# pauxy-qmc/pauxy

Hardware: AMD Instinct MI355X
Metric: walker_steps_per_sec (higher is better)
Workload: dtype f64; 1 GPU; generic Cholesky AFQMC: Nbasis=100, Nchol=500, RHF trial 25+25 electrons, 256 walkers/GPU, dt=0.005, reortho/10, comb/5, energy/10 (BASELINE configs[2]); walkers_total=256, rng=device-philox, population_control=device comb (one rank)

## Files before the change

include/afqmc_hip.h:

```cpp
#ifndef AFQMC_HIP_H
#define AFQMC_HIP_H

#include <stdint.h>

#ifdef __cplusplus
extern "C" {
#endif

typedef struct afq_handle afq_handle;

#define AFQ_OK            0
#define AFQ_EINVAL       (-1)
#define AFQ_ESTATE       (-2)
#define AFQ_EHIP         (-3)
#define AFQ_ENOMEM       (-4)
#define AFQ_EUNSUPPORTED (-5)
#define AFQ_EWEIGHT      (-6)
#define AFQ_EOVERFLOW    (-7)
#define AFQ_ECOMM        (-8)

#define AFQ_SYS_GENERIC 1
#define AFQ_SYS_HUBBARD 2
#define AFQ_SYS_UEG     3

// ... 48 lines not shown
                       const double *vqvec, double vol, const double *H1diag, double ecore);
int afq_set_trial(afq_handle *h, const double *psi);
int afq_set_propagator_hirsch(afq_handle *h, const double *bt2, double dt, int charge_decomposition);
int afq_hirsch_free_projection(afq_handle *h, int on);
int afq_hirsch_single_site(afq_handle *h, int on);
int afq_propagate_hirsch_free(afq_handle *h, const double *u, int32_t *fields_out, double eshift);
int afq_propagate_hirsch(afq_handle *h, double eshift);
int afq_hirsch_kinetic(afq_handle *h);
int afq_hirsch_two_body(afq_handle *h, const double *u, int32_t *fields_out, int32_t *used_out);
int afq_hirsch_finish(afq_handle *h, double eshift);

int afq_local_energy_full_g(afq_handle *h, const double *G, int n, double *E_out);
int afq_ueg_pair_sums(afq_handle *h, const double *G, int n, double *E_out, double *two_rdm_out);
int afq_hubbard_energy_full_g(afq_handle *h, const double *G, int n, double *E_out);

int afq_bp_configure(afq_handle *h, int nbp);
int afq_bp_steps(afq_handle *h, int32_t *steps_out);
int afq_bp_update(afq_handle *h, const double *phi_bp0, int nstblz, int restore_weights, int eval_energy,
                  int reset, double *est_out);
int afq_bp_observables(afq_handle *h, int two_rdm, int ekt, const double *h1, const double *L, int nL);
int afq_bp_ekt_chunks(afq_handle *h, int nc, int ncy);
int afq_bp_update_ext(afq_handle *h, const double *phi_bp0, int nstblz, int restore_weights, int eval_energy,
                      int reset, double *est_out, double *two_rdm_out, double *fock_out);
int afq_bp_update_msd(afq_handle *h, int ndet, const double *dets, const double *coeffs, int nstblz, int restore_weights,
                      int eval_energy, int reset, double *est_out, double *detw_out);

int afq_itcf_configure(afq_handle *h, int nmax, int neqlb, int stable, int restore_weights);
int afq_itcf_update(afq_handle *h, const double *psi_T, int nstblz, double *spgf_out, double *denom_out);

int afq_set_trial_multi(afq_handle *h, int ndet, const double *psi, const double *coeffs, const double *rchol);
int afq_walkers_det_weights(afq_handle *h, double *weights_out);

int afq_set_propagator(afq_handle *h, const double *BH1, const double *mf_shift,
                       double dt, int exp_order, int flags);

int afq_walkers_alloc(afq_handle *h, int nw);
int afq_walkers_set(afq_handle *h, int field, const void *host, int first, int count);
int afq_walkers_get(afq_handle *h, int field, void *host, int first, int count);
int afq_walkers_device_ptr(afq_handle *h, int field, void **dev_ptr, int64_t *bytes_per_walker);

int afq_greens(afq_handle *h, int want_G, double *ovlp_out);
int afq_calc_overlap(afq_handle *h, double *ovlp_out);
int afq_inverse_overlap(afq_handle *h, double *oinv_out, double *ovlp_out);
int afq_propagate(afq_handle *h, const double *xi, double eshift_re, double eshift_im);
int afq_propagate_begin(afq_handle *h, const double *xi);
int afq_propagate_finish(afq_handle *h, double eshift_re, double eshift_im);
int afq_reortho(afq_handle *h, double *detR_out);
int afq_set_log_shift(afq_handle *h, int on, double log_shift, double detR_shift);
int afq_log_ovlp_sums(afq_handle *h, double *sums3);
int afq_local_energy(afq_handle *h, double *E_out);

int afq_set_exchange_algorithm(afq_handle *h, int mode);
int afq_exchange_algorithm(afq_handle *h, int *mode_out);

int afq_set_msd_force_bias(afq_handle *h, int mode);
int afq_msd_force_bias(afq_handle *h, int *mode_out);

int afq_force_bias(afq_handle *h, double *xbar_out);
int afq_shift_fields(afq_handle *h, const double *xi, const double *xbar,
                     double *xs_out, double *cmf_out, double *cfb_out);
int afq_vhs(afq_handle *h, const double *xs, double *vhs_out);
int afq_vhs_count(afq_handle *h, int *nv);
int afq_apply_exponential(afq_handle *h, const double *vhs);
int afq_kinetic(afq_handle *h);

int afq_cap_weights(afq_handle *h, double frac, double total_weight);
int afq_set_weight_cap(afq_handle *h, double frac, double total_weight);
int afq_popcontrol_comb(afq_handle *h, double r, double target_weight,
                        int32_t *parent_ix, double *total_weight_out);

#define AFQ_COMM_ID_BYTES 128
#define AFQ_COMM_NSTATS 12
typedef int (*afq_allgather_fn)(const void *send, void *recv, int bytes, void *user);
int afq_comm_unique_id(void *id_out);
int afq_comm_available(void);
int afq_comm_init(afq_handle *h, const void *unique_id, int rank, int nranks);
int afq_comm_init_ipc(afq_handle *h, int rank, int nranks, afq_allgather_fn allgather, void *user);
int afq_comm_destroy(afq_handle *h);
int afq_comm_set_transport(afq_handle *h, int window);
int afq_comm_set_capacity(afq_handle *h, int max_walkers_per_peer);
int afq_comm_set_timeout(afq_handle *h, double seconds);
int afq_comm_probe(afq_handle *h, int64_t *mismatch_out);
int afq_comm_stats(afq_handle *h, int64_t *out);
int afq_comm_parent_ix(afq_handle *h, int32_t *parent_ix_global);
int afq_estimates_allreduce(afq_handle *h, double *buf, int nest);
int afq_comm_init_local(afq_handle **handles, int n);
int afq_popcontrol_comb_local(afq_handle **handles, int n, double r, double target_weight,
                              int32_t *parent_ix_global, double *total_weight_out);
int afq_estimates_allreduce_local(afq_handle **handles, int n);
int afq_walkers_scale_weights(afq_handle *h, double scale);
int afq_walkers_copy(afq_handle *h, int src, int dst);
int afq_walker_pack_bytes(afq_handle *h, int64_t *bytes);
int afq_walker_pack(afq_handle *h, int iw, void *dev_buf);
int afq_walker_unpack(afq_handle *h, int iw, const void *dev_buf);
int afq_walkers_reset_weights(afq_handle *h);
int afq_estimates_update(afq_handle *h, int eval_energy);
int afq_estimates_rdm(afq_handle *h, int on);
int afq_estimates_sf(afq_handle *h, int on);
int afq_estimates_sf_get(afq_handle *h, double *sf_out , int zero);
int afq_estimates_rdm_get(afq_handle *h, double *rdm_out , int zero);
int afq_estimates_get(afq_handle *h, double *est_out , int zero);
int afq_estimates_fuse_next(afq_handle *h);
int afq_estimates_get_begin(afq_handle *h, int zero);
int afq_estimates_update_publish(afq_handle *h, int eval_energy, int zero);
int afq_estimates_get_end(afq_handle *h, double *est_out );

// ... 30 lines not shown
```

pauxy_amd/_lib.py:

```python
import ctypes
import os
from ctypes import POINTER, c_char_p, c_double, c_int, c_int32, c_int64, c_uint64, c_void_p

HERE = os.path.dirname(os.path.abspath(__file__))
LIB_PATH = os.environ.get("AFQ_LIBRARY") or os.path.join(HERE, "libafqmc_hip.so")

AFQ_OK = 0
AFQ_EWEIGHT, AFQ_EOVERFLOW, AFQ_ECOMM = -6, -7, -8
AFQ_COMM_NSTATS = 12
ALLGATHER_FN = ctypes.CFUNCTYPE(ctypes.c_int, ctypes.c_void_p, ctypes.c_void_p, ctypes.c_int, ctypes.c_void_p)
AFQ_SYS_GENERIC, AFQ_SYS_HUBBARD, AFQ_SYS_UEG = 1, 2, 3
AFQ_PROP_HYBRID, AFQ_PROP_FORCE_BIAS, AFQ_PROP_FREE_PROJECTION, AFQ_PROP_HUBBARD_SPIN = 1, 2, 4, 8
(F_PHI, F_WEIGHT, F_UNSCALED_WEIGHT, F_OT, F_HYBRID_ENERGY, F_PHASE, F_DETR, F_ELOC, F_GHALF, F_G,
 F_XBAR, F_XSHIFTED, F_ENERGY, F_LOG_DETR) = range(14)

_h = c_void_p
_dp = c_void_p
_ip = c_void_p

SIGNATURES = {
    "afq_version": [],
    "afq_create": [c_int, POINTER(_h)],
    "afq_destroy": [_h],
    "afq_last_error": [_h],
# ... 46 lines not shown
    "afq_rng_seed": [_h, c_uint64, c_uint64],
    "afq_counters": [_h, c_void_p, c_int],
    "afq_counters_ext": [_h, c_void_p, c_int, c_int],
    "afq_propagator_issued_flops": [_h, POINTER(c_double), POINTER(c_double)],
    "afq_timers": [_h, _dp, c_int],
    "afq_enable_timers": [_h, c_int],
    "afq_stream": [_h, POINTER(c_void_p)],
    "afq_inverse_overlap": [_h, _dp, _dp],
    "afq_set_propagator_hirsch": [_h, _dp, c_double, c_int],
    "afq_propagate_hirsch": [_h, c_double],
    "afq_hirsch_free_projection": [_h, c_int],
    "afq_hirsch_single_site": [_h, c_int],
    "afq_propagate_hirsch_free": [_h, _dp, c_void_p, c_double],
    "afq_hirsch_kinetic": [_h],
    "afq_hirsch_two_body": [_h, _dp, _dp, _dp],
    "afq_hirsch_finish": [_h, c_double],
    "afq_bp_configure": [_h, c_int],
    "afq_bp_steps": [_h, _dp],
    "afq_bp_update": [_h, _dp, c_int, c_int, c_int, c_int, _dp],
    "afq_bp_observables": [_h, c_int, c_int, _dp, _dp, c_int],
    "afq_bp_ekt_chunks": [_h, c_int, c_int],
    "afq_bp_update_ext": [_h, _dp, c_int, c_int, c_int, c_int, _dp, _dp, _dp],
    "afq_bp_update_msd": [_h, c_int, _dp, _dp, c_int, c_int, c_int, c_int, _dp, _dp],
    "afq_itcf_configure": [_h, c_int, c_int, c_int, c_int],
    "afq_itcf_update": [_h, _dp, c_int, _dp, _dp],
    "afq_local_energy_full_g": [_h, _dp, c_int, _dp],
    "afq_ueg_pair_sums": [_h, _dp, c_int, _dp, _dp],
    "afq_hubbard_energy_full_g": [_h, _dp, c_int, _dp],
    "afq_set_trial_multi": [_h, c_int, _dp, _dp, _dp],
    "afq_walkers_det_weights": [_h, _dp],
    "afq_rng_normal": [_h, _dp, c_int64],
    "afq_rng_philox4x32": [_h, c_void_p, c_void_p, c_int],
    "afq_debug": [_h, c_int, c_int],
    "afq_last_launch": [_h, c_void_p, c_int, POINTER(c_uint64), POINTER(c_uint64)],
    "afq_comm_unique_id": [c_void_p],
    "afq_comm_available": [],
    "afq_comm_init": [_h, c_void_p, c_int, c_int],
    "afq_comm_init_ipc": [_h, c_int, c_int, ALLGATHER_FN, c_void_p],
    "afq_comm_set_transport": [_h, c_int],
    "afq_comm_probe": [_h, c_void_p],
    "afq_comm_destroy": [_h],
    "afq_comm_set_capacity": [_h, c_int],
    "afq_comm_set_timeout": [_h, c_double],
    "afq_launch_trace": [_h, c_int],
    "afq_launch_trace_get": [_h, c_void_p, c_int, c_void_p, c_void_p, c_int, POINTER(c_int)],
    "afq_comm_stats": [_h, c_void_p],
    "afq_comm_parent_ix": [_h, c_void_p],
    "afq_estimates_allreduce": [_h, _dp, c_int],
    "afq_comm_init_local": [POINTER(_h), c_int],
    "afq_popcontrol_comb_local": [POINTER(_h), c_int, c_double, c_double, c_void_p, POINTER(c_double)],
    "afq_estimates_allreduce_local": [POINTER(_h), c_int],
    "afq_set_exchange_algorithm": [_h, c_int],
    "afq_exchange_algorithm": [_h, POINTER(c_int)],
    "afq_set_msd_force_bias": [_h, c_int],
    "afq_msd_force_bias": [_h, POINTER(c_int)],
    "afq_kernel_trace": [_h, c_int],
    "afq_kernel_trace_stride": [_h, c_int, c_int],
    "afq_kernel_trace_get": [_h, c_int, _dp, c_int, POINTER(c_int)],
    "afq_kernel_issued_flops": [_h, c_int, POINTER(c_double)],
}


class AfqLibraryError(RuntimeError):
    pass


class AfqError(RuntimeError):
    def __init__(self, code, text):
        RuntimeError.__init__(self, "libafqmc_hip error %d: %s" % (code, text))
        self.code = code


_lib = None


def load(path=None):
    global _lib
    if _lib is not None and path is None:
        return _lib
    p = path or LIB_PATH
    if not os.path.exists(p):
        raise AfqLibraryError(
            "%s not found: build it with `python -c 'import __graft_entry__ as g; g.build()'` "
            "(or `make -C pauxy_amd/csrc`).  There is no CPU fallback." % p)
    try:
        lib = ctypes.CDLL(p)
    except OSError as e:
        raise AfqLibraryError("cannot load %s: %s" % (p, e))
    for name, args in SIGNATURES.items():
        try:
            fn = getattr(lib, name)
        except AttributeError:
            raise AfqLibraryError("%s does not export %s" % (p, name))
        fn.argtypes = args
        fn.restype = c_char_p if name == "afq_last_error" else c_int
    if path is None:
        _lib = lib
    return lib

K_PROPAGATOR, K_EXCHANGE, K_VHS, K_FORCE_BIAS, K_GREENS = range(5)
```

pauxy_amd/csrc/afq_api.hip:

```cpp
#include <algorithm>
#include <cmath>
#include <complex>
#include <cstdio>
#include <cstdlib>
#include <cstring>
#include "afq_host.h"

namespace {

void free_dets(afq_handle *h) {
    h->mem.release(LT_TRIAL);
    h->dets.assign(1, afq_handle::DetOps());
    h->ndet = 1;
    select_det(h, 0, true);
    h->msd_fb_gbar = false;
}

void free_system(afq_handle *h) {
    free_dets(h);
    h->mem.release(LT_SYSTEM);
    h->hs_cplx = 0; h->sf_nlong = 0; h->kind = 0;
    h->hirsch = false;
}

// ... 921 lines not shown
    const bool keep = kept != GreensCache::NOTHING && h->ndet == 1;
    bool scaled = false;
    { PhaseTimer t(h, T_QR); if ((rc = k_reortho(h, keep ? h->ovlp_new : nullptr, &scaled))) return rc; }
    if (keep) {
        if (!scaled && (rc = k_scale_by_inverse(h, h->ovlp_new, h->detR))) return rc;
        h->gf.keep(kept);
    }
    if (h->log_shift_on && (rc = k_log_shift_reortho(h))) return rc;
    return copy_out(h, detR_out, h->detR, sizeof(double) * h->nw);
}

static int local_energy_dets(afq_handle *h) {
    cplx *final_e = h->energy;
    int rc = AFQ_OK;
    for (int d = 0; d < h->ndet && !rc; ++d) {
        select_det(h, d);
        h->energy = h->energy_all + (size_t)d * 3 * h->nw;
        rc = k_energy_generic(h);
    }
    h->energy = final_e;
    select_det(h, 0);
    return rc;
}

static int local_energy(afq_handle *h) {
    if (h->kind == AFQ_SYS_GENERIC && h->ndet > 1) {
        int rc = local_energy_dets(h);
        if (rc) return rc;
        return k_msd_energy_combine(h);
    }
    if (h->kind == AFQ_SYS_GENERIC) return k_energy_generic(h);
    if (h->kind == AFQ_SYS_HUBBARD) return k_energy_hubbard(h);
    if (!h->G) AFQ_FAIL(h, AFQ_ESTATE, "afq_greens must run before afq_local_energy");
    return k_energy_ueg(h);
}

int afq_local_energy(afq_handle *h, double *E_out) {
    AFQ_API(h, "afq_local_energy");
    if (!h) return AFQ_EINVAL;
    int rc = need_ready(h, false);
    if (rc) return rc;
    if (!h->rH1 && h->kind != AFQ_SYS_UEG) AFQ_FAIL(h, AFQ_ESTATE, "half-rotated H1 missing (set trial)");
    if ((rc = ensure_spin_ghalf(h))) return rc;
    { PhaseTimer t(h, T_ENERGY); if ((rc = local_energy(h))) return rc; }
    return copy_out(h, E_out, h->energy, sizeof(cplx) * 3 * h->nw);
}

int afq_set_exchange_algorithm(afq_handle *h, int mode) {
    if (!h || mode < 0 || mode > 2) return AFQ_EINVAL;
    h->exx_mode = mode;
    return AFQ_OK;
}

int afq_set_msd_force_bias(afq_handle *h, int mode) {
    if (!h || mode < 0 || mode > 2) return AFQ_EINVAL;
    h->msd_fb_mode = mode;
    return AFQ_OK;
}

int afq_msd_force_bias(afq_handle *h, int *mode) {
    if (!h || !mode) return AFQ_EINVAL;
    if (h->kind != AFQ_SYS_GENERIC || !h->have_trial || !h->nw) AFQ_FAIL(h, AFQ_ESTATE, "generic system, trial and walkers must be set");
    *mode = h->ndet <= 1 ? 0 : k_msd_gbar_wanted(h) ? 2 : 1;
    return AFQ_OK;
}

int afq_exchange_algorithm(afq_handle *h, int *mode) {
    if (!h || !mode) return AFQ_EINVAL;
    if (h->kind != AFQ_SYS_GENERIC || !h->have_trial) AFQ_FAIL(h, AFQ_ESTATE, "generic system and trial must be set");
    *mode = k_exchange_uses_quadratic(h) ? 2 : 1;
    return AFQ_OK;
}

int afq_force_bias(afq_handle *h, double *xbar_out) {
    if (!h) return AFQ_EINVAL;
    int rc = need_ready(h, true);
    if (rc) return rc;
    if ((rc = force_bias(h))) return rc;
    return copy_out(h, xbar_out, h->xbar, sizeof(cplx) * (size_t)h->nw * h->K);
}

int afq_shift_fields(afq_handle *h, const double *xi, const double *xbar, double *xs_out, double *cmf_out,
                     double *cfb_out) {
    if (!h || !xi || !xbar) return AFQ_EINVAL;
    int rc = need_ready(h, true);
    if (rc) return rc;
    const size_t n = (size_t)h->nw * h->K;
    AFQ_HIP(h, hipMemcpyAsync(h->xi, xi, sizeof(double) * n, hipMemcpyHostToDevice, h->stream));
    AFQ_HIP(h, hipMemcpyAsync(h->xbar, xbar, sizeof(cplx) * n, hipMemcpyHostToDevice, h->stream));
    if ((rc = k_fields_explicit(h, h->xi, h->xbar, h->xs, h->cmf, h->cfb))) return rc;
    if ((rc = copy_out(h, xs_out, h->xs, sizeof(cplx) * n))) return rc;
    if ((rc = copy_out(h, cmf_out, h->cmf, sizeof(cplx) * h->nw))) return rc;
    return copy_out(h, cfb_out, h->cfb, sizeof(cplx) * h->nw);
}

int afq_vhs_count(afq_handle *h, int *nv) {
    if (!h || !nv) return AFQ_EINVAL;
    *nv = h->nv;
    return AFQ_OK;
}

int afq_vhs(afq_handle *h, const double *xs, double *vhs_out) {
    if (!h || !xs || !vhs_out) return AFQ_EINVAL;
    int rc = need_ready(h, true);
    if (rc) return rc;
    const size_t n = (size_t)h->nw * h->K;
// ... 685 lines not shown
```

pauxy_amd/csrc/afq_internal.h:

```cpp
#pragma once
#include <hip/hip_runtime.h>
#include <stdint.h>
#include <cstdlib>
#include <string>
#include <vector>
#include "../../include/afqmc_hip.h"
#include "greens_cache.h"
#include "dev_mem.h"

typedef double2 cplx;

__host__ __device__ inline cplx cmake(double r, double i) { return make_double2(r, i); }
__host__ __device__ inline cplx cadd(cplx a, cplx b) { return cmake(a.x + b.x, a.y + b.y); }
__host__ __device__ inline cplx csub(cplx a, cplx b) { return cmake(a.x - b.x, a.y - b.y); }
__host__ __device__ inline cplx cmul(cplx a, cplx b) {
    return cmake(a.x * b.x - a.y * b.y, a.x * b.y + a.y * b.x);
}
__host__ __device__ inline cplx cconj(cplx a) { return cmake(a.x, -a.y); }
__host__ __device__ inline cplx cscale(cplx a, double s) { return cmake(a.x * s, a.y * s); }
__host__ __device__ inline void cfma(cplx &a, cplx b, cplx c) {
    a.x = fma(b.x, c.x, a.x); a.x = fma(-b.y, c.y, a.x);
    a.y = fma(b.x, c.y, a.y); a.y = fma(b.y, c.x, a.y);
}
__host__ __device__ inline double cabs2(cplx a) { return a.x * a.x + a.y * a.y; }
__device__ inline cplx cdiv(cplx a, cplx b) {
    if (fabs(b.x) >= fabs(b.y)) {
        double r = b.y / b.x, d = b.x + b.y * r;
        return cmake((a.x + a.y * r) / d, (a.y - a.x * r) / d);
    } else {
        double r = b.x / b.y, d = b.x * r + b.y;
        return cmake((a.x * r + a.y) / d, (a.y * r - a.x) / d);
    }
}

#define AFQ_NSCAL 12
enum { AFQ_HS_HERMITIAN = 1, AFQ_HS_GENERAL = 2 };
enum { T_GREENS = 0, T_ONEBODY, T_FB, T_VHS, T_EXP, T_OVLP, T_QR, T_ENERGY, T_COUNT };

#define AFQ_NCOUNTERS 8

struct afq_handle {
    int device = 0;
    hipStream_t stream = nullptr;
    std::string err;
    DevMem mem;

    int kind = 0;
    int M = 0, K = 0, na = 0, nb = 0, nt = 0;
    double ecore = 0.0;
    double *hs_pot = nullptr;
    bool hs_sym = false;
    double *L_full = nullptr;
    int2 *hs_pair = nullptr;
    int hs_cplx = 0;
    double *hs_pot_im = nullptr;
    int2 *hs_pair_im = nullptr;
    long ld_hs_im = 0;
    cplx *L_full_c = nullptr;
    long ld_hs = 0, ld_rc = 0;
    bool rchol_real = true;
    double *rchol_re = nullptr;
    double *rchol_im = nullptr;
    double *rchol_frag[2] = {nullptr, nullptr};
    double *rchol_frag_im[2] = {nullptr, nullptr};
    void *atil[2] = {nullptr, nullptr};
    bool atil_unavailable = false;
    bool rchol_same = false;
    int exx_mode = 0;
    cplx *exq_y = nullptr;
    size_t exq_y_len = 0;
    cplx *H1 = nullptr;
    cplx *rH1 = nullptr;
    double U = 0.0;
    int nq = 0;
    int64_t nnzA = 0, nnzB = 0;
    int64_t *iA_colptr = nullptr, *iA_row = nullptr; cplx *iA_val = nullptr;
    int64_t *iB_colptr = nullptr, *iB_row = nullptr; cplx *iB_val = nullptr;
    int64_t *iA_rowptr = nullptr, *iA_col = nullptr; cplx *iA_rval = nullptr;
    int64_t *iB_rowptr = nullptr, *iB_col = nullptr; cplx *iB_rval = nullptr;
    int ell_len = 0; int *ell_row = nullptr; cplx *ell_val = nullptr;
    int ueg_nrows = 0; int *ueg_rmap = nullptr; int *ueg_rows = nullptr;
    int *ueg_kp = nullptr, *ueg_pm = nullptr, *ueg_koff = nullptr, *ueg_poff = nullptr;
    int64_t *kpq_off = nullptr, *kpq_i = nullptr, *kpq_kpq = nullptr;
    int64_t *pmq_off = nullptr, *pmq_i = nullptr, *pmq_pmq = nullptr;
    double *vqvec = nullptr; double vol = 1.0; double *H1diag = nullptr;
    void *ueg_fast = nullptr;
    int *sf_kp = nullptr, *sf_pm = nullptr, *sf_order = nullptr;
    int sf_nlong = 0;
    cplx *sf_ws = nullptr, *sf_two = nullptr;
    size_t sf_ws_len = 0, sf_two_len = 0;

    bool have_trial = false;
    cplx *psi = nullptr;
    cplx *psic = nullptr;
    cplx *psicT = nullptr;
    long psi_stride = 0;
    bool psi_real = false;
    bool psi_closed = false;
    unsigned long long *closed_bad = nullptr;
    unsigned long long closed_epoch = 0;
    unsigned long long closed_epoch_pub = 0;
    bool exx_open_hint = false;
    int *closed_w = nullptr;
    size_t closed_w_n = 0;
    bool closed_large = false;

    struct DetOps {
        cplx *psi = nullptr, *psic = nullptr, *rH1 = nullptr;
        double *rchol_re = nullptr, *rchol_im = nullptr;
        double *rchol_frag[2] = {nullptr, nullptr}, *rchol_frag_im[2] = {nullptr, nullptr};
        void *atil[2] = {nullptr, nullptr};
        bool rchol_same = false;
        GreensCache::Stamp vbias_stamp;
    };
    int ndet = 1, cur_det = 0;
    std::vector<DetOps> dets = std::vector<DetOps>(1);
    cplx *coeffs = nullptr;
    cplx *detd = nullptr;
    cplx *detd_a = nullptr;
    cplx *detw = nullptr;
    cplx *ghalf_all = nullptr;
// ... 245 lines not shown
    }
}

struct PhaseTimer {
    afq_handle *h; int slot;
    PhaseTimer(afq_handle *h_, int s) : h(h_), slot(s) {
        if (h->timers_on) hipEventRecord(h->ev0, h->stream);
    }
    ~PhaseTimer() {
        if (h->timers_on) {
            hipEventRecord(h->ev1, h->stream);
            hipEventSynchronize(h->ev1);
            float ms = 0; hipEventElapsedTime(&ms, h->ev0, h->ev1);
            h->t_ms[slot] += ms;
        }
    }
};

template <class T> struct Lent {
    T &slot; T saved;
    Lent(T &s, T v) : slot(s), saved(s) { slot = v; }
    ~Lent() { slot = saved; }
    Lent(const Lent &) = delete;
    Lent &operator=(const Lent &) = delete;
};

struct KernelTrace {
    afq_handle *h; int kind, idx;
    KernelTrace(afq_handle *h_, int k) : h(h_), kind(k), idx(-1) {
        if (!(h->ktrace_mask >> k & 1) || h->ktrace_used[k] >= 4096) return;
        if (h->ktrace_seen[k]++ % h->ktrace_stride[k]) return;
        idx = h->ktrace_used[k];
        std::vector<hipEvent_t> &ev = h->ktrace_ev[k];
        while ((int)ev.size() < 2 * idx + 2) { hipEvent_t e; hipEventCreate(&e); ev.push_back(e); }
        hipEventRecord(ev[2 * idx], h->stream);
    }
    ~KernelTrace() {
        if (idx < 0) return;
        hipEventRecord(h->ktrace_ev[kind][2 * idx + 1], h->stream);
        h->ktrace_used[kind] = idx + 1;
    }
};

int k_onebody(afq_handle *h, const cplx *rowscale = nullptr);
int k_force_bias_generic(afq_handle *h);
bool k_msd_vbias_current(afq_handle *h);
bool k_msd_gbar_wanted(afq_handle *h);
int k_force_bias_msd_gbar(afq_handle *h);
bool k_fb_use_sum(afq_handle *h);
int k_vhs_generic(afq_handle *h);
int k_apply_exponential(afq_handle *h, const cplx *vhs);
int k_full_G(afq_handle *h);
int k_prop_fused_supported(afq_handle *h);
int k_prop_fused(afq_handle *h);
int k_hirsch_alive(afq_handle *h, int mode);
int k_hirsch_kinetic(afq_handle *h);
int k_hirsch_two_body(afq_handle *h);
int k_hirsch_eshift(afq_handle *h, double fac);
int k_hirsch_free(afq_handle *h, double eshift);
int k_rng_uniform(afq_handle *h, double *u, long n);
int k_energy_full_g(afq_handle *h, const cplx *G_dev, int ng, cplx *E_dev);
int k_fullg_expand(afq_handle *h);
int k_bp_observables(afq_handle *h, int restore, cplx *two_out, cplx *fock_out);
int k_itcf_fields(afq_handle *h, cplx *xs, int t);
int k_itcf_generic_b(afq_handle *h, const cplx *vhs, const cplx *BT2, const cplx *BT2inv, cplx *B, cplx *Binv, cplx *ws,
                     cplx *detm, int *dete);
int k_itcf_hirsch_b(afq_handle *h, int t, const cplx *BT2, const cplx *BT2inv, cplx *B, cplx *Binv, double *f);
int k_itcf_mul(afq_handle *h, const cplx *A, const cplx *B, cplx *C);
int k_itcf_propagate(afq_handle *h, const cplx *B, const cplx *src, cplx *dst);
int k_itcf_projectors(afq_handle *h, const cplx *G, cplx *P, cplx *Q);
int k_itcf_weights(afq_handle *h, int restore, cplx *wfac, cplx *denom);
int k_itcf_accumulate(afq_handle *h, const cplx *Ggr, const cplx *Gls, const cplx *wfac, cplx *spgf_tau);
int k_greens_big_supported(afq_handle *h);
int k_greens_big(afq_handle *h, cplx *ghalf, cplx *det, cplx *oinv, const GreensRequest &req, GreensResult *res);
int k_reortho_big(afq_handle *h);
int k_gj_inverse(afq_handle *h, cplx *O, int n, int batch, cplx *detm, int *dete);
int k_alive(afq_handle *h);
int k_greens(afq_handle *h, cplx *det_out, const GreensRequest &req = GreensRequest(), GreensResult *res = nullptr);
int k_overlap(afq_handle *h, cplx *det_out, const GreensRequest &req = GreensRequest(), GreensResult *res = nullptr);
int k_inverse_overlap(afq_handle *h, cplx *oinv, cplx *det_out);
int k_fields(afq_handle *h);
int k_fields_explicit(afq_handle *h, const double *xi_d, const cplx *xbar_d, cplx *xs_d, cplx *cmf_d, cplx *cfb_d);
int k_xbar(afq_handle *h);
int k_bp_push(afq_handle *h);
int k_bp_fields(afq_handle *h, int i);
int k_bp_init(afq_handle *h, const cplx *phi0_dev);
int k_conj_copy(afq_handle *h, const cplx *src, cplx *dst, long n);
int k_conj_transpose(afq_handle *h, const cplx *A, cplx *At);
int k_bp_accumulate(afq_handle *h, int restore, int with_energy);
int k_bp_reset(afq_handle *h, bool first);
int k_bp_hirsch_step(afq_handle *h, int i);
int k_bp_msd_onebody(afq_handle *h, int ndet, const cplx *src, cplx *dst);
int k_bp_msd_taylor(afq_handle *h, int ndet, const cplx *vhs, cplx *phi, cplx *t0, cplx *t1);
int k_bp_msd_logr(afq_handle *h, const double *detR, double *logr, long n);
int k_bp_msd_detw(afq_handle *h, int ndet, int d, const cplx *coeffs, const double *logr, const cplx *ovlp, cplx *detw,
                  cplx *S);
int k_bp_msd_gsum(afq_handle *h, int ndet, int d, const cplx *detw, const cplx *G, cplx *gsum, const cplx *E, cplx *esum);
int k_bp_msd_finish(afq_handle *h, int ndet, int restore, cplx *detw, const cplx *S, cplx *fac);
int k_bp_msd_accumulate(afq_handle *h, const cplx *gsum, const cplx *fac, const cplx *esum, cplx *est);
int k_xbar_fields(afq_handle *h, cplx *hubbard_factors = nullptr);
int k_msd_combine(afq_handle *h, cplx *det_out, bool skip_small);
int k_msd_energy_combine(afq_handle *h);
int k_update_weight(afq_handle *h, cplx eshift);
struct WeightArgs;
WeightArgs k_weight_args(afq_handle *h, cplx eshift);
int k_reortho(afq_handle *h, cplx *keep = nullptr, bool *keep_done = nullptr);
// ... 52 lines not shown
```

pauxy_amd/csrc/k_fused.hip:

```cpp
#include <cstdlib>
#include <type_traits>

#include "mfma_gemm_wg.h"

#define PF_D 3
#ifndef PF_NW
#define PF_NW 8
#endif
#define PF_NT (64 * PF_NW)
#ifndef PF_LW
#define PF_LW PF_NW
#endif
#define PF_FPW (16 / PF_LW)

struct PropFusedArgs {
    int M, na, nb, nt, order;
    int vhs_upper;
    int same_b;
    int b_real;
    int rem4;
    int hyb;
    int symcols;
    int closed_try;
    int contig;
    const cplx *BH1;
    const cplx *vhs;
    cplx *phi;
    const int *alive;
    const void *zero16;
    unsigned long long *n_closed;
};

__device__ inline d2_t lds_read_c(unsigned addr) { return lds_read_b128(addr); }

template <int OFF> __device__ inline d2_t lds_read_off(unsigned addr) {
    d2_t v;
    asm volatile("ds_read_b128 %0, %1 offset:%2" : "=v"(v) : "v"(addr), "n"(OFF));
    return v;
}
__device__ __attribute__((always_inline)) inline d2_t lds_read_frag(unsigned base, int idx) {
    switch (idx) {
    case 0: return lds_read_off<0>(base);
    case 1: return lds_read_off<1024>(base);
    case 2: return lds_read_off<2048>(base);
    case 3: return lds_read_off<3072>(base);
    case 4: return lds_read_off<4096>(base);
    case 5: return lds_read_off<5120>(base);
    case 6: return lds_read_off<6144>(base);
    default: return lds_read_off<7168>(base);
    }
}

template <int OFF> __device__ inline double lds_read_re_off(unsigned addr) {
    double v;
    asm volatile("ds_read_b64 %0, %1 offset:%2" : "=v"(v) : "v"(addr), "n"(OFF));
    return v;
}
__device__ __attribute__((always_inline)) inline double lds_read_frag_re(unsigned base, int idx) {
    switch (idx) {
    case 0: return lds_read_re_off<0>(base);
    case 1: return lds_read_re_off<1024>(base);
    case 2: return lds_read_re_off<2048>(base);
    case 3: return lds_read_re_off<3072>(base);
    case 4: return lds_read_re_off<4096>(base);
    case 5: return lds_read_re_off<5120>(base);
    case 6: return lds_read_re_off<6144>(base);
    default: return lds_read_re_off<7168>(base);
    }
}

__device__ inline void lds_barrier() {
    asm volatile("s_waitcnt lgkmcnt(0)" ::: "memory");
    __builtin_amdgcn_s_barrier();
    asm volatile("" ::: "memory");
}

template <bool NARROW, int FULL>
__global__ __launch_bounds__(PF_NT) void prop_fused_kernel(PropFusedArgs a) {
    extern __shared__ __align__(16) unsigned char smem[];
    const int w = blockIdx.x;
    if (!a.alive[w]) return;
    const int tid = threadIdx.x, lane = tid & 63, wave = __builtin_amdgcn_readfirstlane(tid >> 6);
    const int lr = lane & 15, lk = lane >> 4;
    const int M = a.M, nt = a.nt;
    const int NCH = (M + 7) >> 3;
    const int nrt = (M + 15) >> 4;
    unsigned char *Tf = smem;
    unsigned char *ring = smem + (size_t)NCH * 8192;
    const unsigned tf_l = lds_addr(Tf), ring_l = lds_addr(ring);
    cplx *phi = a.phi + (long)w * M * nt;
    const cplx *vhs = a.vhs + (long)w * M * M;

    const int nob = a.same_b ? 1 : 2;
    const int nphase = 2 * nob + a.order;
    const int G = nphase * NCH;
    const long MM = (long)M * M;
    int gi = 0, gi_phase = 0, gi_c = 0, gi_slot = 0;
    const void *nsrc[PF_FPW];
    bool prepared = false;
    const bool refills = wave >= PF_NW - PF_LW;
    const int lw = wave - (PF_NW - PF_LW);
    const int p_row0 = (lw >> 1) * 16 + lr;
    const int p_kl = 2 * lk + (lw & 1);
    auto prepare = [&]() __attribute__((always_inline)) {
        if (!refills) { prepared = true; return; }
        const bool in_v = gi_phase >= nob && gi_phase < nob + a.order;
        const int spin = gi_phase < nob ? gi_phase : gi_phase - nob - a.order;
        const cplx *A = in_v ? vhs : a.BH1 + (spin == 1 ? MM : 0L);
        const bool sym_phase = a.vhs_upper && in_v;
        const bool live = gi < G;
        const int k = gi_c * 8 + p_kl;
#pragma unroll
        for (int t = 0; t < PF_FPW; ++t) {
            const int row = p_row0 + t * (PF_LW / 2) * 16;
            const int off = (sym_phase && k < row) ? k * M + row : row * M + k;
            nsrc[t] = (live && row < M && k < M) ? (const void *)(A + off) : a.zero16;
            asm volatile("" : "+v"(nsrc[t]));
        }
        ++gi;
        const bool wrap = gi_c + 1 == NCH;
        gi_c = wrap ? 0 : gi_c + 1;
        gi_phase += wrap ? 1 : 0;
        prepared = true;
    };
    auto issueA = [&]() __attribute__((always_inline)) {
        if (!refills) return;
        if (!prepared) prepare();
        unsigned char *dst = ring + (size_t)gi_slot * 16384;
#pragma unroll
        for (int t = 0; t < PF_FPW; ++t) glds16(nsrc[t], dst + (lw + t * PF_LW) * 1024);
        if (++gi_slot == PF_D) gi_slot = 0;
        prepared = false;
    };
    issueA(); issueA();
    prepare();
    bool closed = false;
    if (a.closed_try) {
        bool same = true;
        for (int p = tid >> 5; p < M; p += PF_NT / 32) {
            const int c = tid & 31;
            if (c < a.na) {
                const cplx x = phi[p * nt + c], y = phi[p * nt + a.na + c];
                same = same && __double_as_longlong(x.x) == __double_as_longlong(y.x) &&
                       __double_as_longlong(x.y) == __double_as_longlong(y.y);
            }
        }
        closed = __builtin_amdgcn_readfirstlane(__syncthreads_and(same ? 1 : 0)) != 0;
        if (closed && tid == 0) atomicAdd(a.n_closed, 1ULL);
    }
    const bool relayout = closed && a.contig;
    const int contig = relayout ? 0 : a.contig, hyb = relayout ? 0 : a.hyb;
    const int sym_n = (a.symcols && !relayout) ? a.na : 0;
    auto wcol = [&](const int c) -> int {
        if (!sym_n) return c;
        if (c < 16) return c;
        if (c < 32) return sym_n + (c - 16);
        if (c < 40) return 16 + (c - 32);
        if (c < 48) return sym_n + 16 + (c - 40);
        const int e = c - 48, extra = sym_n - 24;
        return e < extra ? 24 + e : sym_n + 24 + (e - extra);
    };

    for (int e = tid; e < NCH * 512; e += PF_NT) {
        const int j = e & 15, kk = (e >> 4) & 3, pb = (e >> 6) & 1, slot = (e >> 7) & 3, ch = e >> 9;
        const int p = ch * 8 + 2 * kk + pb, sp = contig ? 0 : slot >> 1, col = (contig ? slot : slot & 1) * 16 + j;
        const int ns_ = contig ? nt : sp ? a.nb : a.na, off_ = sp ? a.na : 0;
        const bool ok = p < M && col < ns_;
        const cplx v = phi[ok ? p * nt + off_ + wcol(col) : 0];
        ((d2_t *)Tf)[e] = ok ? (d2_t){v.x, v.y} : (d2_t){0.0, 0.0};
    }
    __syncthreads();

    auto t_ok = [&](int ti, int r) -> bool { return 2 * ti + (r >> 1) < NCH; };
    const unsigned t_lane = (unsigned)((lk & 1) * 1024 + ((lk >> 1) * 16 + lr) * 16);
    auto t_addr = [&](int ti, int r, int cs) -> unsigned {
        unsigned base = t_lane;
        asm volatile("" : "+v"(base));
        return base + (unsigned)(((2 * ti * 4 + cs) * 2) * 1024) + (unsigned)((r >> 1) * 8192 + (r & 1) * 512);
    };

    int ring_slot = 0;
    auto next_chunk = [&]() __attribute__((always_inline)) -> unsigned {
        asm volatile("s_waitcnt vmcnt(%0)" ::"n"((PF_D - 2) * PF_FPW) : "memory");
        __builtin_amdgcn_s_barrier();
        issueA();
        const unsigned sl = ring_l + ring_slot * 16384;
        if (++ring_slot == PF_D) ring_slot = 0;
        return sl;
    };
    auto next_chunk_sync = [&]() __attribute__((always_inline)) -> unsigned {
        asm volatile("s_waitcnt vmcnt(%0)" ::"n"((PF_D - 2) * PF_FPW) : "memory");
        __builtin_amdgcn_s_barrier();
        const unsigned sl = ring_l + ring_slot * 16384;
        ring_slot = ring_slot + 1 == PF_D ? 0 : ring_slot + 1;
        return sl;
    };

    auto one_body = [&](auto nsl_tag, int slot0, bool to_global, auto real_tag, const int rt) __attribute__((always_inline)) {
        constexpr int NSL = decltype(nsl_tag)::value;
        constexpr bool BR = decltype(real_tag)::value;
        constexpr int SS = (NARROW && FULL) ? 2 : 1;
// ... 710 lines not shown
        else if (nrt <= 6) taylor(I2{}, I1{}, std::true_type{}, 4 + (wave & 1), 2 * ((wave - 4) >> 1), 1, std::false_type{});
        else taylor(I2{}, I1{}, std::true_type{}, (wave & 1) ? 6 : 4, 2 * ((wave - 4) >> 1), (wave & 1) ? 1 : 2, std::false_type{});
    }
    else if (FULL == 7 && contig) {
        if constexpr (FULL == 7) {
            using I1 = std::integral_constant<int, 1>;
            using I2 = std::integral_constant<int, 2>;
            auto deal = [&](auto nu) __attribute__((always_inline)) {
                if (wave == 0 || wave == 2) taylor(I2{}, I2{}, std::false_type{}, wave, 0, 2, std::false_type{});
                else if (wave == 1 || wave == 3) taylor_h(std::true_type{}, std::false_type{}, nu, wave - 1, 2, 3, 0);
                else if (wave == 4 || wave == 6) taylor(I1{}, I1{}, std::true_type{}, 4, (wave - 4) >> 1, 1, std::true_type{});
                else if (wave == 5) taylor(I1{}, I2{}, std::true_type{}, 5, 0, 1, std::false_type{});
                else taylor_h(std::true_type{}, std::true_type{}, nu, 4, 2, 3, 2);
            };
            if (hyb == 2) deal(I2{});
            else deal(I1{});
        }
    }
    else if (FULL >= 5 && closed) {
        using I1 = std::integral_constant<int, 1>;
        using I2 = std::integral_constant<int, 2>;
        const int cs = wave & 1;
        if (wave < 4) taylor(I2{}, I1{}, std::false_type{}, 2 * (wave >> 1), cs, 2, std::false_type{});
        else if constexpr (FULL == 7) {
            if (a.rem4) {
                if (wave < 6) taylor(I1{}, I1{}, std::true_type{}, 4, cs, 1, std::true_type{});
                else taylor(I1{}, I1{}, std::true_type{}, 5, cs, 1, std::false_type{});
            } else {
                if (wave < 6) taylor(I2{}, I1{}, std::true_type{}, 4, cs, 2, std::false_type{});
                else taylor(I1{}, I1{}, std::true_type{}, 6, cs, 1, std::false_type{});
            }
        }
        else taylor(I1{}, I1{}, std::true_type{}, (FULL == 6 && wave >= 6) ? 5 : 4, cs, 1, std::false_type{});
        mirror_spin();
    }
    else if (wave < 4) taylor(std::integral_constant<int, 2>{}, std::integral_constant<int, 2>{}, std::false_type{}, 2 * (wave >> 1), 2 * (wave & 1), 2, std::false_type{});
    else if constexpr (FULL == 7) {
        if (a.rem4) taylor(std::integral_constant<int, 2>{}, std::integral_constant<int, 1>{}, std::true_type{}, 4, wave - 4, 2, std::true_type{});
        else taylor(std::integral_constant<int, 3>{}, std::integral_constant<int, 1>{}, std::true_type{}, 4, wave - 4, 3, std::false_type{});
    }
    else if (FULL >= 5) taylor(std::integral_constant<int, FULL >= 5 ? FULL - 4 : 1>{}, std::integral_constant<int, 1>{}, std::true_type{}, 4, wave - 4, FULL - 4, std::false_type{});
    else taylor(std::integral_constant<int, 3>{}, std::integral_constant<int, 1>{}, std::true_type{}, 4, wave - 4, 3, std::false_type{});
#endif
    if (a.order == 0) lds_barrier();

    one_body_stage(true);
    asm volatile("s_waitcnt vmcnt(0)" ::: "memory");
}

int k_prop_fused_supported(afq_handle *h) {
    return !h->vhs_diag && h->nv == 1 && h->M <= 104 && h->na <= 32 && h->nb <= 32 && h->nb > 0;
}

int k_prop_fused(afq_handle *h) {
    PropFusedArgs a;
    a.M = h->M; a.na = h->na; a.nb = h->nb; a.nt = h->nt; a.order = h->exp_order;
    a.vhs_upper = h->vhs_upper ? 1 : 0;
    a.same_b = h->bh1_same ? 1 : 0;
    a.b_real = h->bh1_real ? 1 : 0;
    a.rem4 = (h->M > 96 && h->M <= 100) ? 1 : 0;
    a.hyb = 0;
    a.contig = 0; a.symcols = 0;
    if (a.rem4 && a.same_b && h->na > 16 && h->nb > 16 && h->nt > 48 && h->nt <= 56 && PF_NW == 8) {
        a.contig = 1;
        a.hyb = (h->nt - 48 + 3) / 4;
    }
    a.symcols = (a.contig && h->na == h->nb) ? 1 : 0;
    a.closed_try = 0;
    a.BH1 = h->BH1; a.vhs = h->vhs; a.phi = h->phi; a.alive = h->alive; a.zero16 = h->zero_page;
    a.n_closed = h->counters + 3;
    const int NCH = (h->M + 7) / 8;
    const size_t lds = (size_t)NCH * 8192 + (size_t)PF_D * 16384;
    static size_t lds_set[6][AFQ_MAX_DEVICES] = {{0}, {0}, {0}, {0}, {0}, {0}};
    const bool narrow = h->na <= 16 && h->nb <= 16;
    KernelTrace kt(h, AFQ_K_PROPAGATOR);
    {
        const int nrt_ = (h->M + 15) / 16, ct = (h->na + 15) / 16 + (h->nb + 15) / 16;
        const double ksteps = 2.0 * NCH;
        const double per_pass = ksteps * (2048.0 * (a.rem4 ? nrt_ - 1 : nrt_) * ct + 512.0 * (a.rem4 ? ct : 0));
        const double taylor_pass = a.contig ? ksteps * (2048.0 * (nrt_ - 1) * 3 + 512.0 * (nrt_ - 1) * a.hyb + 512.0 * 4) : per_pass;
        h->issued_flops[AFQ_K_PROPAGATOR] = (3.0 * h->exp_order * taylor_pass + 2.0 * (a.b_real ? 2.0 : 3.0) * per_pass) * h->nw;
        h->prop_issued_open = h->issued_flops[AFQ_K_PROPAGATOR] / h->nw;
        const int cta = (h->na + 15) / 16;
        const double closed_pass = ksteps * (2048.0 * (a.rem4 ? nrt_ - 1 : nrt_) * cta + 512.0 * (a.rem4 ? cta : 0));
        h->prop_issued_closed = 3.0 * h->exp_order * closed_pass + 2.0 * (a.b_real ? 2.0 : 3.0) * per_pass;
    }
    const int nrt = (h->M + 15) / 16;
    const bool nofull = PF_NW != 8;
    const int full = nofull ? 0 : narrow ? (nrt == 6 ? 6 : 0) : (nrt >= 5 && h->na > 16 && h->nb > 16 ? nrt : 0);
    a.closed_try = (a.same_b && h->na == h->nb && h->exp_order > 0 && full != 0 && PF_NW == 8 &&
                    (!a.contig || a.symcols)) ? 1 : 0;
#define PF_LAUNCH_(NARROW_, FULL_, SLOT_)                                                                     \
    do {                                                                                                      \
        AFQ_HIP(h, afq_raise_lds((const void *)prop_fused_kernel<NARROW_, FULL_>, lds, lds_set[SLOT_]));      \
        AFQ_LAUNCH(h, (prop_fused_kernel<NARROW_, FULL_>), dim3(h->nw), dim3(PF_NT), lds, h->stream, a);      \
    } while (0)
    if (narrow && full) PF_LAUNCH_(true, 6, 0);
    else if (narrow) PF_LAUNCH_(true, 0, 1);
    else if (full == 7) PF_LAUNCH_(false, 7, 2);
    else if (full == 6) PF_LAUNCH_(false, 6, 3);
    else if (full == 5) PF_LAUNCH_(false, 5, 4);
    else PF_LAUNCH_(false, 0, 5);
#undef PF_LAUNCH_
    AFQ_POST(h);
    return AFQ_OK;
}
```

pauxy_amd/device.py:

```python
import ctypes

import numpy

from pauxy_amd import _lib as L


def _c128(a, shape=None):
    a = numpy.ascontiguousarray(a, dtype=numpy.complex128)
    if shape is not None:
        assert a.shape == tuple(shape), (a.shape, shape)
    return a


def _f64(a, shape=None):
    a = numpy.ascontiguousarray(a, dtype=numpy.float64)
    if shape is not None:
        assert a.shape == tuple(shape), (a.shape, shape)
    return a


def _i64(a):
    return numpy.ascontiguousarray(a, dtype=numpy.int64)


# ... 528 lines not shown
                         'reortho', 'energy'], out))

    def kernel_trace(self, on=True, kinds=None):
        arg = int(bool(on))
        if on and kinds is not None:
            arg = sum(2 << int(k) for k in kinds)
        self._ck(self.lib.afq_kernel_trace(self.h, arg))

    def kernel_trace_stride(self, kind, stride):
        self._ck(self.lib.afq_kernel_trace_stride(self.h, int(kind), int(stride)))

    def kernel_trace_get(self, kind, max_n=4096):
        out = numpy.zeros(max_n, dtype=numpy.float64)
        n = ctypes.c_int()
        self._ck(self.lib.afq_kernel_trace_get(self.h, int(kind), _p(out), max_n, ctypes.byref(n)))
        return out[:min(n.value, max_n)]

    def launch_trace(self, on=True):
        self._ck(self.lib.afq_launch_trace(self.h, int(bool(on))))

    def launch_trace_get(self):
        cap = 256
        names = ctypes.create_string_buffer(cap * 96)
        ms = numpy.zeros(cap, dtype=numpy.float64)
        cnt = numpy.zeros(cap, dtype=numpy.int64)
        n = ctypes.c_int()
        self._ck(self.lib.afq_launch_trace_get(self.h, ctypes.cast(names, ctypes.c_void_p), len(names), _p(ms), _p(cnt),
                                               cap, ctypes.byref(n)))
        out, at = {}, 0
        for k in range(min(n.value, cap)):
            end = names.raw.index(b'\0', at)
            out[names.raw[at:end].decode()] = (int(cnt[k]), float(ms[k]))
            at = end + 1
        return out

    def kernel_issued_flops(self, kind):
        out = ctypes.c_double(0.0)
        self._ck(self.lib.afq_kernel_issued_flops(self.h, int(kind), ctypes.byref(out)))
        return float(out.value)

    def propagator_issued_flops(self):
        a, b = ctypes.c_double(0.0), ctypes.c_double(0.0)
        self._ck(self.lib.afq_propagator_issued_flops(self.h, ctypes.byref(a), ctypes.byref(b)))
        return float(a.value), float(b.value)

    def set_exchange_algorithm(self, mode):
        self._ck(self.lib.afq_set_exchange_algorithm(self.h, int(mode)))

    def exchange_algorithm(self):
        m = ctypes.c_int()
        self._ck(self.lib.afq_exchange_algorithm(self.h, ctypes.byref(m)))
        return m.value

    def set_msd_force_bias(self, mode):
        self._ck(self.lib.afq_set_msd_force_bias(self.h, int(mode)))

    def msd_force_bias(self):
        m = ctypes.c_int()
        self._ck(self.lib.afq_msd_force_bias(self.h, ctypes.byref(m)))
        return m.value


def _handle_array(devs):
    return (ctypes.c_void_p * len(devs))(*[d.h.value for d in devs])


def comm_init_local(devs):
    lib = devs[0].lib
    rc = lib.afq_comm_init_local(_handle_array(devs), len(devs))
    if rc != 0:
        raise L.AfqError(rc, lib.afq_last_error(devs[0].h).decode())
    for i, d in enumerate(devs):
        d.comm_rank, d.comm_size = i, len(devs)


def popcontrol_comb_local(devs, r, target, fetch=True):
    lib = devs[0].lib
    n = len(devs)
    if not fetch:
        rc = lib.afq_popcontrol_comb_local(_handle_array(devs), n, float(r), float(target), None, None)
        pix = tw = None
    else:
        pix = numpy.zeros(n * devs[0].nw, dtype=numpy.int32)
        tw = ctypes.c_double(0.0)
        rc = lib.afq_popcontrol_comb_local(_handle_array(devs), n, float(r), float(target), _p(pix), ctypes.byref(tw))
        tw = tw.value
    if rc != 0:
        raise L.AfqError(rc, lib.afq_last_error(devs[0].h).decode())
    return pix, tw


def estimates_allreduce_local(devs):
    lib = devs[0].lib
    rc = lib.afq_estimates_allreduce_local(_handle_array(devs), len(devs))
    if rc != 0:
        raise L.AfqError(rc, lib.afq_last_error(devs[0].h).decode())
```

Measured before the change: 1.035 million walker-steps/s.

## Add register-resident closed-shell propagator path for the fused kernel

```diff
diff --git a/include/afqmc_hip.h b/include/afqmc_hip.h
--- a/include/afqmc_hip.h
+++ b/include/afqmc_hip.h
@@ -124,6 +124,9 @@
 
 int afq_set_exchange_algorithm(afq_handle *h, int mode);
 int afq_exchange_algorithm(afq_handle *h, int *mode_out);
+
+int afq_set_propagator_closed_form(afq_handle *h, int mode);
+int afq_propagator_closed_form(afq_handle *h, int *mode_out);
 
 int afq_set_msd_force_bias(afq_handle *h, int mode);
 int afq_msd_force_bias(afq_handle *h, int *mode_out);
diff --git a/pauxy_amd/_lib.py b/pauxy_amd/_lib.py
--- a/pauxy_amd/_lib.py
+++ b/pauxy_amd/_lib.py
@@ -122,6 +122,8 @@
     "afq_estimates_allreduce_local": [POINTER(_h), c_int],
     "afq_set_exchange_algorithm": [_h, c_int],
     "afq_exchange_algorithm": [_h, POINTER(c_int)],
+    "afq_set_propagator_closed_form": [_h, c_int],
+    "afq_propagator_closed_form": [_h, POINTER(c_int)],
     "afq_set_msd_force_bias": [_h, c_int],
     "afq_msd_force_bias": [_h, POINTER(c_int)],
     "afq_kernel_trace": [_h, c_int],
diff --git a/pauxy_amd/csrc/afq_api.hip b/pauxy_amd/csrc/afq_api.hip
--- a/pauxy_amd/csrc/afq_api.hip
+++ b/pauxy_amd/csrc/afq_api.hip
@@ -997,6 +997,18 @@
     return AFQ_OK;
 }
 
+int afq_set_propagator_closed_form(afq_handle *h, int mode) {
+    if (!h || mode < 0 || mode > 2) return AFQ_EINVAL;
+    h->prop_closed_mode = mode;
+    return AFQ_OK;
+}
+
+int afq_propagator_closed_form(afq_handle *h, int *mode) {
+    if (!h || !mode) return AFQ_EINVAL;
+    *mode = k_prop_closed_resident(h) ? 2 : 1;
+    return AFQ_OK;
+}
+
 int afq_set_msd_force_bias(afq_handle *h, int mode) {
     if (!h || mode < 0 || mode > 2) return AFQ_EINVAL;
     h->msd_fb_mode = mode;
diff --git a/pauxy_amd/csrc/afq_internal.h b/pauxy_amd/csrc/afq_internal.h
--- a/pauxy_amd/csrc/afq_internal.h
+++ b/pauxy_amd/csrc/afq_internal.h
@@ -67,6 +67,7 @@
     bool atil_unavailable = false;
     bool rchol_same = false;
     int exx_mode = 0;
+    int prop_closed_mode = 0;
     cplx *exq_y = nullptr;
     size_t exq_y_len = 0;
     cplx *H1 = nullptr;
@@ -418,6 +419,7 @@
 int k_apply_exponential(afq_handle *h, const cplx *vhs);
 int k_full_G(afq_handle *h);
 int k_prop_fused_supported(afq_handle *h);
+int k_prop_closed_resident(afq_handle *h);
 int k_prop_fused(afq_handle *h);
 int k_hirsch_alive(afq_handle *h, int mode);
 int k_hirsch_kinetic(afq_handle *h);
diff --git a/pauxy_amd/csrc/k_fused.hip b/pauxy_amd/csrc/k_fused.hip
--- a/pauxy_amd/csrc/k_fused.hip
+++ b/pauxy_amd/csrc/k_fused.hip
@@ -29,6 +29,7 @@
     const int *alive;
     const void *zero16;
     unsigned long long *n_closed;
+    int resident;
 };
 
 __device__ inline d2_t lds_read_c(unsigned addr) { return lds_read_b128(addr); }
@@ -74,6 +75,8 @@
     __builtin_amdgcn_s_barrier();
     asm volatile("" ::: "memory");
 }
+
+#include "k_fused_closed.h"
 
 template <bool NARROW, int FULL>
 __global__ __launch_bounds__(PF_NT) void prop_fused_kernel(PropFusedArgs a) {
@@ -147,6 +150,13 @@
         }
         closed = __builtin_amdgcn_readfirstlane(__syncthreads_and(same ? 1 : 0)) != 0;
         if (closed && tid == 0) atomicAdd(a.n_closed, 1ULL);
+    }
+    if constexpr (!NARROW && FULL == 7 && PF_NW == 8) {
+        if (closed && a.resident) {
+            if (M <= 100) prop_closed_resident<25>(a, smem, phi, vhs);
+            else prop_closed_resident<26>(a, smem, phi, vhs);
+            return;
+        }
     }
     const bool relayout = closed && a.contig;
     const int contig = relayout ? 0 : a.contig, hyb = relayout ? 0 : a.hyb;
@@ -963,6 +973,11 @@
     return !h->vhs_diag && h->nv == 1 && h->M <= 104 && h->na <= 32 && h->nb <= 32 && h->nb > 0;
 }
 
+int k_prop_closed_resident(afq_handle *h) {
+    return PF_NW == 8 && k_prop_fused_supported(h) && h->prop_closed_mode != 1 && h->bh1_same && h->bh1_real &&
+           h->na == h->nb && h->na > 16 && h->na <= 32 && h->M > 96 && h->M <= 104 && h->exp_order > 0;
+}
+
 int k_prop_fused(afq_handle *h) {
     PropFusedArgs a;
     a.M = h->M; a.na = h->na; a.nb = h->nb; a.nt = h->nt; a.order = h->exp_order;
@@ -995,12 +1010,15 @@
         const int cta = (h->na + 15) / 16;
         const double closed_pass = ksteps * (2048.0 * (a.rem4 ? nrt_ - 1 : nrt_) * cta + 512.0 * (a.rem4 ? cta : 0));
         h->prop_issued_closed = 3.0 * h->exp_order * closed_pass + 2.0 * (a.b_real ? 2.0 : 3.0) * per_pass;
+        if (k_prop_closed_resident(h))
+            h->prop_issued_closed = (4.0 * h->exp_order + 2.0 * 2.0) * ((h->M + 3) / 4) * 2048.0 * 7 * 2;
     }
     const int nrt = (h->M + 15) / 16;
     const bool nofull = PF_NW != 8;
     const int full = nofull ? 0 : narrow ? (nrt == 6 ? 6 : 0) : (nrt >= 5 && h->na > 16 && h->nb > 16 ? nrt : 0);
     a.closed_try = (a.same_b && h->na == h->nb && h->exp_order > 0 && full != 0 && PF_NW == 8 &&
                     (!a.contig || a.symcols)) ? 1 : 0;
+    a.resident = (a.closed_try && full == 7 && k_prop_closed_resident(h)) ? 1 : 0;
 #define PF_LAUNCH_(NARROW_, FULL_, SLOT_)                                                                     \
     do {                                                                                                      \
         AFQ_HIP(h, afq_raise_lds((const void *)prop_fused_kernel<NARROW_, FULL_>, lds, lds_set[SLOT_]));      \
diff --git a/pauxy_amd/csrc/k_fused_closed.h b/pauxy_amd/csrc/k_fused_closed.h
--- /dev/null
+++ b/pauxy_amd/csrc/k_fused_closed.h
@@ -0,0 +1,134 @@
+#pragma once
+
+#define PCR_LDS(p) ((__attribute__((address_space(3))) unsigned char *)(p))
+
+template <int KS>
+__device__ __attribute__((always_inline)) inline void prop_closed_resident(const PropFusedArgs &a, unsigned char *smem_,
+                                                                           cplx *phi, const cplx *vhs) {
+    auto *smem = PCR_LDS(smem_);
+    typedef __attribute__((address_space(3))) d2_t lds_d2;
+    const int tid = threadIdx.x, wave = __builtin_amdgcn_readfirstlane(tid >> 6);
+    const int M = a.M, nt = a.nt, na = a.na;
+    constexpr unsigned TB = KS * 2048;
+    const bool mul = wave < 7;
+    auto lane_id = [&]() __attribute__((always_inline)) -> int {
+        int t = tid;
+        asm volatile("" : "+v"(t));
+        return t & 63;
+    };
+
+    for (int e = tid; e < KS * 128; e += PF_NT) {
+        const int k = 4 * (e >> 7) + ((e >> 4) & 3), col = 16 * ((e >> 6) & 1) + (e & 15);
+        const bool ok = k < M && col < na;
+        const cplx v = phi[ok ? k * nt + col : 0];
+        ((lds_d2 *)smem)[e] = ok ? (d2_t){v.x, v.y} : (d2_t){0.0, 0.0};
+    }
+    __syncthreads();
+
+    auto load_b = [&](double (&bh)[KS]) __attribute__((always_inline)) {
+        const int lane = lane_id(), lk = lane >> 4, row = wave * 16 + (lane & 15);
+#pragma unroll
+        for (int s = 0; s < KS; ++s) {
+            const int k = 4 * s + lk;
+            const double *p = (row < M && k < M) ? &a.BH1[row * M + k].x : (const double *)a.zero16;
+            bh[s] = *p;
+        }
+    };
+    auto one_body = [&](const unsigned src, const double (&bh)[KS], d4_t (&P1)[2], d4_t (&P2)[2]) __attribute__((always_inline)) {
+#pragma unroll
+        for (int j = 0; j < 2; ++j) { P1[j] = (d4_t){0, 0, 0, 0}; P2[j] = (d4_t){0, 0, 0, 0}; }
+        const auto *tb = smem + src + lane_id() * 16;
+#pragma unroll
+        for (int s = 0; s < KS; ++s) {
+#pragma unroll
+            for (int j = 0; j < 2; ++j) {
+                const d2_t b = *(const lds_d2 *)(tb + (s * 2 + j) * 1024);
+                P1[j] = mfma16(bh[s], b[0], P1[j]);
+                P2[j] = mfma16(bh[s], b[1], P2[j]);
+            }
+        }
+    };
+    auto put = [&](const unsigned dst, const d4_t (&re)[2], const d4_t (&im)[2]) __attribute__((always_inline)) {
+        auto *tb = smem + dst + lane_id() * 16;
+#pragma unroll
+        for (int q = 0; q < 4; ++q)
+            if (4 * wave + q < KS) {
+#pragma unroll
+                for (int j = 0; j < 2; ++j) *(lds_d2 *)(tb + ((4 * wave + q) * 2 + j) * 1024) = (d2_t){re[j][q], im[j][q]};
+            }
+    };
+
+    d2_t av[KS];
+    d4_t SR[2], SI[2];
+    if (mul) {
+        double bh[KS];
+        load_b(bh);
+        const int lane = lane_id(), lk = lane >> 4, row = wave * 16 + (lane & 15);
+#pragma unroll
+        for (int s = 0; s < KS; ++s) {
+            const int k = 4 * s + lk;
+            const int off = (a.vhs_upper && k < row) ? k * M + row : row * M + k;
+            const d2_t *p = (row < M && k < M) ? (const d2_t *)(vhs + off) : (const d2_t *)a.zero16;
+            av[s] = *p;
+        }
+        one_body(0, bh, SR, SI);
+        put(TB, SR, SI);
+    }
+    lds_barrier();
+
+    unsigned cur = TB;
+    for (int n = 1; n <= a.order; ++n) {
+        if (mul) {
+            double inv_n = 1.0 / n;
+            asm volatile("" : "+v"(inv_n));
+            d4_t P1[2], P2[2], P3[2];
+#pragma unroll
+            for (int j = 0; j < 2; ++j) { P1[j] = (d4_t){0, 0, 0, 0}; P2[j] = (d4_t){0, 0, 0, 0}; P3[j] = (d4_t){0, 0, 0, 0}; }
+            const auto *tb = smem + cur + lane_id() * 16;
+#pragma unroll
+            for (int s = 0; s < KS; ++s) {
+                asm volatile("" : "+v"(av[s]));
+#pragma unroll
+                for (int j = 0; j < 2; ++j) {
+                    const d2_t b = *(const lds_d2 *)(tb + (s * 2 + j) * 1024);
+                    P3[j] = mfma16(av[s][0], b[1], P3[j]);
+                    P1[j] = mfma16(av[s][0], b[0], P1[j]);
+                    P2[j] = mfma16(av[s][1], b[1], P2[j]);
+                    P3[j] = mfma16(av[s][1], b[0], P3[j]);
+                }
+            }
+            d4_t re[2], im[2];
+#pragma unroll
+            for (int j = 0; j < 2; ++j)
+#pragma unroll
+                for (int q = 0; q < 4; ++q) {
+                    re[j][q] = (P1[j][q] - P2[j][q]) * inv_n;
+                    im[j][q] = P3[j][q] * inv_n;
+                    SR[j][q] += re[j][q]; SI[j][q] += im[j][q];
+                }
+            if (n == a.order) put(cur ^ TB, SR, SI);
+            else put(cur ^ TB, re, im);
+        }
+        lds_barrier();
+        cur ^= TB;
+    }
+
+    if (mul) {
+        d4_t P1[2], P2[2];
+        double bh[KS];
+        load_b(bh);
+        one_body(cur, bh, P1, P2);
+        const int lane = lane_id(), lr = lane & 15, lk = lane >> 4;
+#pragma unroll
+        for (int j = 0; j < 2; ++j)
+#pragma unroll
+            for (int q = 0; q < 4; ++q) {
+                const int orow = wave * 16 + lk + 4 * q, col = 16 * j + lr;
+                if (orow < M && col < na) {
+                    const cplx v = cmake(P1[j][q], P2[j][q]);
+                    phi[(long)orow * nt + col] = v;
+                    phi[(long)orow * nt + na + col] = v;
+                }
+            }
+    }
+}
diff --git a/pauxy_amd/device.py b/pauxy_amd/device.py
--- a/pauxy_amd/device.py
+++ b/pauxy_amd/device.py
@@ -604,6 +604,14 @@
         self._ck(self.lib.afq_exchange_algorithm(self.h, ctypes.byref(m)))
         return m.value
 
+    def set_propagator_closed_form(self, mode):
+        self._ck(self.lib.afq_set_propagator_closed_form(self.h, int(mode)))
+
+    def propagator_closed_form(self):
+        m = ctypes.c_int()
+        self._ck(self.lib.afq_propagator_closed_form(self.h, ctypes.byref(m)))
+        return m.value
+
     def set_msd_force_bias(self, mode):
         self._ck(self.lib.afq_set_msd_force_bias(self.h, int(mode)))
 
```

After: 1.069 million walker-steps/s (median of 6 runs). 3.3% higher.
